# Zelana-Labs/zelana

Measured on AMD Instinct MI355X. Metric: BN254 G1 MSM Mpoint-scalar/s + L2 proofs/sec at 1/2/4/8 MI355X, higher is better.
Workload: dtype u32

## Files before the change

### zelana_amd/csrc/dev_io.h

```cpp
#pragma once
#include <hip/hip_runtime.h>

#include "ff.h"

namespace zk {

__device__ __forceinline__ Fe ld_fe(const uint32_t* p) {
  uint4 a = reinterpret_cast<const uint4*>(p)[0];
  uint4 b = reinterpret_cast<const uint4*>(p)[1];
  uint32_t w[8] = {a.x, a.y, a.z, a.w, b.x, b.y, b.z, b.w};
  return unpack(w);
}
__device__ __forceinline__ void st_fe(uint32_t* p, const Fe& f) {
  uint32_t w[8];
  pack(w, f);
  reinterpret_cast<uint4*>(p)[0] = make_uint4(w[0], w[1], w[2], w[3]);
  reinterpret_cast<uint4*>(p)[1] = make_uint4(w[4], w[5], w[6], w[7]);
}
__device__ __forceinline__ Fe ldc_fe(const uint32_t* c) {
  uint32_t w[8];
#pragma unroll
  for (int i = 0; i < 8; i++) w[i] = c[i];
  return unpack(w);
}

}
```

### zelana_amd/csrc/ec.h

```cpp
#pragma once
#include "ff.h"

#if defined(__HIPCC__) || defined(__HIP__)
#define ZK_HD_NOINLINE __host__ __device__ __noinline__
#else
#define ZK_HD_NOINLINE inline
#endif

namespace zk {


template <class F>
struct Aff {
  typename F::T x, y;
};
template <class F>
struct Xyzz {
  typename F::T x, y, zz, zzz;
};

template <class F>
ZK_HD Xyzz<F> xyzz_inf() {
  Xyzz<F> r;
  r.x = F::zero();
// ... 190 lines not shown
  r.zzz = f2_mul_n(p.zzz, ppp);
  return r;
}

template <class P = FqP>
ZK_HD Xyzz<FqOps> xyzz_add_g1(const Xyzz<FqOps>& p, const Xyzz<FqOps>& q) {
  if (xyzz_is_inf(p)) return q;
  if (xyzz_is_inf(q)) return p;
  Fe u1 = mul<P>(p.x, q.zz);
  Fe u2 = mul<P>(q.x, p.zz);
  Fe s1 = mul<P>(p.y, q.zzz);
  Fe s2 = mul<P>(q.y, p.zzz);
  Fe pp_ = subk<P, 2>(u2, u1);
  Fe ny1 = subk<P, 2>(fe_zero(), s1);
  Fe rr = add_lazy(s2, ny1);
  Fe pp = sqr<P>(pp_);
  if (is_zero<P>(pp)) {
    Fe rn = reduce8<P>(subk<P, 2>(s2, s1));
    if (is_zero<P>(rn)) return xyzz_dbl(p);
    return xyzz_inf<FqOps>();
  }
  Fe ppp = mul<P>(pp_, pp);
  Fe qq = mul<P>(u1, pp);
  Fe t = add_lazy(add_lazy(ppp, qq), qq);
  Xyzz<FqOps> r;
  Fe x = subk<P, 6>(sqr<P>(rr), t);
  Fe qx = subk<P, 8>(qq, x);
  r.y = mul2<P>(rr, qx, ny1, ppp);
  r.x = reduce8<P>(x);
  r.zz = mul<P>(mul<P>(p.zz, q.zz), pp);
  r.zzz = mul<P>(mul<P>(p.zzz, q.zzz), ppp);
  return r;
}
ZK_HD Xyzz<Fq2Ops> xyzz_add_g2(const Xyzz<Fq2Ops>& p, const Xyzz<Fq2Ops>& q) {
  if (xyzz_is_inf(p)) return q;
  if (xyzz_is_inf(q)) return p;
  Fe2 u1 = f2_mul_n(p.x, q.zz), u2 = f2_mul_n(q.x, p.zz);
  Fe2 s1 = f2_mul_n(p.y, q.zzz), s2 = f2_mul_n(q.y, p.zzz);
  Fe2 pp_ = {subk<FqPn, 2>(u2.c0, u1.c0), subk<FqPn, 2>(u2.c1, u1.c1)};
  Fe2 rr = {subk<FqPn, 2>(s2.c0, s1.c0), subk<FqPn, 2>(s2.c1, s1.c1)};
  Fe2 pp = f2_sqr_n(pp_);
  if (f2_is_zero(pp)) {
    if (is_zero<FqPn>(reduce8<FqPn>(rr.c0)) && is_zero<FqPn>(reduce8<FqPn>(rr.c1))) return xyzz_dbl(p);
    return xyzz_inf<Fq2Ops>();
  }
  Fe2 r2 = f2_sqr_n(rr);
  Fe2 ppp = f2_mul_n(pp_, pp), qq = f2_mul_n(u1, pp);
  Xyzz<Fq2Ops> r;
  r.x.c0 = reduce8<FqPn>(subk<FqPn, 6>(r2.c0, add_lazy(add_lazy(ppp.c0, qq.c0), qq.c0)));
  r.x.c1 = reduce8<FqPn>(subk<FqPn, 6>(r2.c1, add_lazy(add_lazy(ppp.c1, qq.c1), qq.c1)));
  Fe2 qx = {subk<FqPn, 2>(qq.c0, r.x.c0), subk<FqPn, 2>(qq.c1, r.x.c1)};
  Fe ny0 = subk<FqPn, 2>(fe_zero(), s1.c0), ny1 = subk<FqPn, 2>(fe_zero(), s1.c1);
  Fe nqx1 = subk<FqPn, 4>(fe_zero(), qx.c1), nppp1 = subk<FqPn, 2>(fe_zero(), ppp.c1);
  r.y.c0 = mul4<FqPn>(rr.c0, qx.c0, rr.c1, nqx1, ny0, ppp.c0, ny1, nppp1);
  r.y.c1 = mul4<FqPn>(rr.c0, qx.c1, rr.c1, qx.c0, ny0, ppp.c1, ny1, ppp.c0);
  r.zz = f2_mul_n(f2_mul_n(p.zz, q.zz), pp);
  r.zzz = f2_mul_n(f2_mul_n(p.zzz, q.zzz), ppp);
  return r;
}

ZK_HD Fe fq_cneg(const Fe& y, bool neg_) {
  Fe n = subk<FqP, 2>(fe_zero(), y);
  Fe r;
#pragma unroll
  for (int i = 0; i < NL; i++) r.v[i] = neg_ ? n.v[i] : y.v[i];
  return r;
// ... 38 lines not shown
```

### zelana_amd/csrc/groth16.hip

```cpp
#include <string.h>

#include <algorithm>
#include <unordered_map>
#include <vector>

#include "dev_io.h"
#include "ec.h"
#include "fq_sqrt.h"
#include "r1cs_row.h"
#include "zkmi_internal.h"

struct zkmi_pk {
  zkmi_ctx* ctx;
  uint64_t n = 0, num_instance = 0, num_witness = 0;
  uint32_t log_n = 0;
  uint64_t alpha_g1[8], beta_g1[8], delta_g1[8];
  uint64_t beta_g2[16], gamma_g2[16], delta_g2[16];
  std::vector<uint64_t> gamma_abc;
  uint64_t a0[8], b1_0[8], b2_0[16];
  zkmi_bases *a_query = nullptr, *b_g1_query = nullptr, *b_g2_query = nullptr, *h_query_rev = nullptr,
             *l_query = nullptr;
  zkmi_bases *b_g1_c = nullptr, *b_g2_c = nullptr;
  uint32_t* d_bidx = nullptr;
  size_t nb_c = 0;
// ... 123 lines not shown
  Aff<Fq2Ops> P = {x, y};
  Xyzz<Fq2Ops> acc = xyzz_inf<Fq2Ops>();
  for (int bit = 253; bit >= 0; bit--) {
    acc = xyzz_dbl(acc);
    if ((FR_MOD64_G[bit >> 6] >> (bit & 63)) & 1) acc = xyzz_madd(acc, P);
  }
  if (!xyzz_is_inf(acc)) {
    atomicOr(bad, 2u);
    return;
  }
  st_fe(o, canon_q(x.c0));
  st_fe(o + 8, canon_q(x.c1));
  st_fe(o + 16, canon_q(y.c0));
  st_fe(o + 24, canon_q(y.c1));
}

__global__ void __launch_bounds__(256) k_permute_rev(const uint32_t* __restrict__ in, uint32_t logn, size_t cnt,
                                                     uint32_t* __restrict__ out) {
  size_t p = blockIdx.x * (size_t)blockDim.x + threadIdx.x;
  if (p >= cnt) return;
  size_t src = logn ? (__brev((uint32_t)p) >> (32 - logn)) : 0;
  for (int k = 0; k < 16; k++) out[p * 16 + k] = in[src * 16 + k];
}

__global__ void __launch_bounds__(256) k_to_mont_fr(const uint32_t* __restrict__ z, size_t n, uint32_t* __restrict__ zm,
                                                    size_t zstr = 0) {
  size_t i = blockIdx.x * (size_t)blockDim.x + threadIdx.x;
  if (i >= n) return;
  z += (size_t)blockIdx.y * zstr;
  zm += (size_t)blockIdx.y * n * 8;
  st_fe(zm + i * 8, to_mont<FrP>(ld_fe(z + i * 8)));
}
constexpr uint32_t MATVEC_SHORT = 8;
__device__ __forceinline__ Fe fe_shfl_xor(const Fe& a, int m) {
  Fe r;
#pragma unroll
  for (int i = 0; i < NL; i++) r.v[i] = (uint32_t)__shfl_xor((int)a.v[i], m, 64);
  return r;
}
__device__ __forceinline__ Fe fr_sum_reduce(Fe a) {
#pragma unroll
  for (int i = 0; i < NL - 1; i++) {
    a.v[i + 1] += a.v[i] >> 29;
    a.v[i] &= LMASK;
  }
  return reduce_q32<FrP>(a);
}
template <bool DICT>
__device__ __forceinline__ Fe mv_term(uint64_t k, const uint64_t* __restrict__ col, const uint32_t* __restrict__ val,
                                      const uint2* __restrict__ cv, const uint32_t* __restrict__ coef,
                                      const uint32_t* __restrict__ zm, const uint32_t* __restrict__ zc) {
  if constexpr (DICT) {
    const uint2 e = cv[k];
    Fe t = ld_fe(zc + (size_t)e.x * 8);
    if (e.y) t = mul<FrP>(ld_fe(coef + (size_t)e.y * 8), t);
    return t;
  } else {
    return mul<FrP>(ld_fe(val + k * 8), ld_fe(zm + col[k] * 8));
  }
}
template <bool DICT, class RP>
__global__ void __launch_bounds__(256) k_matvec(const RP* __restrict__ rowptr, const uint64_t* __restrict__ col,
                                                const uint32_t* __restrict__ val, const uint2* __restrict__ cv,
                                                const uint32_t* __restrict__ coef, const uint32_t* __restrict__ zm,
                                                const uint32_t* __restrict__ zc, size_t m, size_t l, size_t n,
                                                int is_a, const uint32_t* __restrict__ lrow, uint32_t nlong, int g,
                                                uint32_t nsb, uint32_t* __restrict__ out, size_t zstr,
                                                size_t zmstr) {
  zc += (size_t)blockIdx.y * zstr;
  if (!DICT) zm += (size_t)blockIdx.y * zmstr;
  out += (size_t)blockIdx.y * n * 8;
  if (blockIdx.x < nsb) {
// ... 1720 lines not shown
```

### zelana_amd/csrc/msm.hip

```cpp
#include <stdarg.h>
#include <stdlib.h>
#include <stdio.h>
#include <string.h>

#include <algorithm>
#include <string>
#include <type_traits>
#include <utility>
#include <vector>
#include <chrono>

#include "dev_io.h"
#include "ec.h"
#include "zkmi_internal.h"

namespace zk {

#define ZK_TAIL_WAVE() __builtin_amdgcn_s_setprio(3)

struct G1T {
  using F = FqOps;
  using P = FqP;
  static constexpr int CW = 8;
  static constexpr int PW = 16;
// ... 28 lines not shown

template <class G>
__device__ __forceinline__ Aff<typename G::F> ld_aff(const uint32_t* bases, uint32_t idx) {
  const uint32_t* p = bases + (size_t)idx * G::PW;
  Aff<typename G::F> a;
  a.x = Io<typename G::F>::ld(p);
  a.y = Io<typename G::F>::ld(p + G::CW);
  return a;
}
template <class G>
__device__ __forceinline__ Xyzz<typename G::F> ld_xyzz(const uint32_t* p) {
  using F = typename G::F;
  Xyzz<F> r;
  r.x = Io<F>::ld(p);
  r.y = Io<F>::ld(p + G::CW);
  r.zz = Io<F>::ld(p + 2 * G::CW);
  r.zzz = Io<F>::ld(p + 3 * G::CW);
  return r;
}
template <class G>
__device__ __forceinline__ void st_xyzz(uint32_t* p, const Xyzz<typename G::F>& v) {
  using F = typename G::F;
  Io<F>::st(p, v.x);
  Io<F>::st(p + G::CW, v.y);
  Io<F>::st(p + 2 * G::CW, v.zz);
  Io<F>::st(p + 3 * G::CW, v.zzz);
}


template <class G>
__device__ __forceinline__ Xyzz<typename G::F> br_add(const Xyzz<typename G::F>& p, const Xyzz<typename G::F>& q) {
  if constexpr (G::CW == 8) return xyzz_add_g1<typename G::P>(p, q);
  else return xyzz_add_g2(p, q);
}

__host__ __device__ constexpr int msm_windows(int c) { return (254 + c - 1) / c + ((254 % c) == 0 ? 1 : 0); }

template <int C, bool BAL>
struct WinLayout {
  static constexpr int W = msm_windows(C);
  static constexpr int A = BAL ? (254 - W * (C - 1) > 0 ? 254 - W * (C - 1) : 0) : W;
  static_assert(A >= 0 && A <= W && (!BAL || A < W), "balanced layout");
  static constexpr int width(int w) { return w < A ? C : C - 1; }
  static constexpr int offset(int w) { return w <= A ? w * C : A * C + (w - A) * (C - 1); }
};

template <int C, bool BAL = false>
__device__ __forceinline__ void scalar_digits(const uint32_t* __restrict__ scalars, size_t i, int32_t* d) {
  uint4 a = reinterpret_cast<const uint4*>(scalars)[2 * i];
  uint4 b = reinterpret_cast<const uint4*>(scalars)[2 * i + 1];
  uint32_t s[9] = {a.x, a.y, a.z, a.w, b.x, b.y, b.z, b.w & 0x3FFFFFFFu, 0};
  using L = WinLayout<C, BAL>;
  constexpr int W = L::W;
  uint32_t carry = 0;
#pragma unroll
  for (int w = 0; w < W; w++) {
      const int bit = L::offset(w), wi = bit >> 5, sh = bit & 31, wd = L::width(w);
    const uint32_t half = 1u << (wd - 1);
    uint64_t v64 = (((uint64_t)s[wi + 1 < 9 ? wi + 1 : 8]) << 32) | s[wi < 9 ? wi : 8];
    uint32_t v = (uint32_t)(v64 >> sh) & ((1u << wd) - 1);
    v += carry;
    if (w < W - 1 && v > half) {
      d[w] = (int32_t)v - (int32_t)(1u << wd);
      carry = 1;
    } else {
      d[w] = (int32_t)v;
// ... 1157 lines not shown
                   uint32_t tskip, uint32_t* __restrict__ buckets, uint32_t* __restrict__ xpts) {
  acc_items_body<G2T>(items, nover, nmain, sval, bases, tn, tskip, buckets, xpts);
}

__global__ void __launch_bounds__(256) k_items_place(const uint4* __restrict__ stage, uint32_t NLO, uint32_t cap,
                                                     const uint32_t* __restrict__ ghist, uint32_t* __restrict__ gcur,
                                                     uint4* __restrict__ items, uint32_t nmain) {
  ZK_TAIL_WAVE();
  __shared__ uint32_t lh[ITEM_CAP_MAX + 1], lstart[ITEM_CAP_MAX + 1], base[ITEM_CAP_MAX + 1], tmp[4];
  const uint32_t h = blockIdx.x;
  const uint4* st = stage + (size_t)h * NLO;
  for (uint32_t c = threadIdx.x; c <= cap; c += 256) lh[c] = 0;
  __syncthreads();
  for (uint32_t x = threadIdx.x; x < NLO; x += 256) {
    const uint4 it = st[x];
    atomicAdd(&lh[min(it.y - it.x, cap)], 1u);
  }
  __syncthreads();
  block_prefix<256>(cap + 1, [&](uint32_t k) { return lh[cap - k]; }, lstart, tmp);
  block_prefix<256>(cap + 1, [&](uint32_t k) { return ghist[cap - k]; }, base, tmp);
  for (uint32_t k = threadIdx.x; k <= cap; k += 256) {
    const uint32_t c = cap - k;
    if (lh[c]) base[k] += atomicAdd(&gcur[c], lh[c]);
  }
  __syncthreads();
  for (uint32_t x = threadIdx.x; x < NLO; x += 256) {
    const uint4 it = st[x];
    const uint32_t k = cap - min(it.y - it.x, cap);
    const uint32_t dst = base[k] + (x - lstart[k]);
    if (dst < nmain) items[dst] = it;
  }
}

template <class G, bool CHUNKED = false>
__global__ void __launch_bounds__(256) k_split_combine(const uint4* __restrict__ split,
                                                       const uint32_t* __restrict__ nsplit,
                                                       const uint32_t* __restrict__ xpts,
                                                       uint32_t* __restrict__ buckets) {
  ZK_TAIL_WAVE();
  using F = typename G::F;
  constexpr int XW = 4 * G::CW;
  constexpr uint32_t BIG = 256;
  __shared__ Xyzz<F> sh[4][32];
  __shared__ uint4 spl[4];
  const uint32_t ns = *nsplit;
  const uint32_t wave = threadIdx.x >> 6, lane = threadIdx.x & 63;
  for (uint32_t base = blockIdx.x * 4; base < ns; base += gridDim.x * 4) {
    if (lane == 0) spl[wave] = base + wave < ns ? split[base + wave] : make_uint4(0, 0, 0, 0);
    __syncthreads();
    uint32_t mxs = 0;
    for (int w = 0; w < 4; w++) mxs = max(mxs, spl[w].z <= BIG ? spl[w].z : 0u);
    const uint32_t nload0 = (mxs + 63) / 64;
    uint32_t lev0 = 0;
    while ((1u << lev0) < min(mxs, 64u)) lev0++;
    const uint4 mine = spl[wave];
    const bool small = mine.z <= BIG;
    Xyzz<F> v = xyzz_inf<F>();
    int ph = 0;
    uint32_t st0 = 0;
    uint32_t nload = nload0, lev = lev0, cross = 0, stride = 64;
    uint4 cur = mine;
    bool mine_in = small;
    for (uint32_t step = 0;; step++) {
      uint32_t k = step - st0;
      if (k >= nload + lev + cross) {
        if (ph == 0) {
          if (small && mine.z && lane == 0) st_xyzz<G>(buckets + (size_t)mine.x * XW, v);
        } else if (threadIdx.x == 0) {
          st_xyzz<G>(buckets + (size_t)cur.x * XW, v);
        }
        v = xyzz_inf<F>();
        int w = ph;
        while (w < 4 && spl[w].z <= BIG) w++;
        if (w >= 4) break;
        ph = w + 1;
        cur = spl[w];
        mine_in = true;
        st0 = step;
        k = 0;
// ... 151 lines not shown
    if (!first_open) {
      ykey[2 * t + 1] = first_key;
      yvalid[2 * t + 1] = 0;
    }
    if (!last_open || (first_key == last_key && first_open)) {
      ykey[2 * t + 2] = last_key;
      yvalid[2 * t + 2] = 0;
    }
    if (t == 0) {
      ykey[0] = first_key;
      yvalid[0] = 0;
    }
  }
  if (!head) return;
  const bool left_open = r == 0 && first_open;
  const bool right_open = key == last_key && last_open;
  if (left_open || right_open) {
    const uint32_t slot = left_open ? 2 * t + 1 : 2 * t + 2;
    ykey[slot] = key;
    yvalid[slot] = has;
    if (has) {
      st_xyzz<G>(ypts + (size_t)slot * XW, v);
      atomicOr(any_open, 1u);
    }
  } else if (has) {
    st_xyzz<G>(buckets + (size_t)key * XW, v);
  }
}


__device__ __forceinline__ uint32_t insert_bit(uint32_t t, int bit) {
  return (((t >> bit) << (bit + 1)) | (1u << bit) | (t & ((1u << bit) - 1)));
}
#define ZK_BR_WPE 4
#ifndef ZK_BR_MINW
#define ZK_BR_MINW 1
#endif

template <class G, bool BITS>
__global__ void __launch_bounds__(256) __attribute__((amdgpu_waves_per_eu(ZK_BR_MINW, ZK_BR_WPE))) k_msm_br(const uint32_t* __restrict__ src0, const uint32_t* __restrict__ src1,
                                                const uint32_t* __restrict__ bstart, int lb, int hb, int W, int sr,
                                                int sc, int sb, int segt, uint32_t* __restrict__ out0,
                                                uint32_t* __restrict__ out1) {
  ZK_TAIL_WAVE();
  using F = typename G::F;
  constexpr int XW = 4 * G::CW;
  __shared__ Xyzz<F> sh[4][32];
  const int bb = lb + hb;
  const uint32_t wave = threadIdx.x >> 6, lane = threadIdx.x & 63;
  const uint32_t job = blockIdx.x * 4 + wave;
  const uint32_t nrow = ((uint32_t)W << hb) * sr, ncol = ((uint32_t)W << lb) * sc;
  const uint32_t njobs = BITS ? (uint32_t)W * (bb + 1) * sb : nrow + ncol;
  const bool live = job < njobs;
  const uint32_t* src = src0;
  uint32_t cnt = 0, stride = 1, bucket0 = 0, t0 = 0;
  int bit = -1, seg = 1;
  uint32_t* dst = nullptr;
  bool canon = false;
  if (live) {
    if (!BITS) {
      if (job < nrow) {
        uint32_t rh = job / sr, g = job % sr, w = rh >> hb, h = rh & ((1u << hb) - 1);
        cnt = (1u << lb) / sr;
        bucket0 = (w << bb) + (h << lb) + g * cnt;
        stride = 1;
        dst = out0 + (size_t)job * XW;
      } else {
        uint32_t jj = job - nrow, cl = jj / sc, g = jj % sc, w = cl >> lb, l = cl & ((1u << lb) - 1);
        cnt = (1u << hb) / sc;
        bucket0 = (w << bb) + ((g * cnt) << lb) + l;
        stride = 1u << lb;
        dst = out1 + (size_t)jj * XW;
      }
      src = src0 + (size_t)bucket0 * XW;
    } else {
      const uint32_t wj = job / sb;
      t0 = (job % sb) * (uint32_t)segt;
      uint32_t w = wj / (bb + 1), j = wj % (bb + 1);
      if ((int)j < lb) {
        src = src1 + (((size_t)w << lb) * sc) * XW;
        cnt = (1u << (lb - 1)) * sc;
        bit = (int)j;
        seg = sc;
      } else if ((int)j < bb) {
        src = src0 + (((size_t)w << hb) * sr) * XW;
        cnt = (1u << (hb - 1)) * sr;
        bit = (int)j - lb;
        seg = sr;
      } else {
        src = src0 + (((size_t)w << hb) * sr) * XW;
        cnt = (1u << hb) * sr;
        seg = sr;
      }
      dst = out0 + (size_t)job * XW;
      canon = true;
    }
  }
  const uint32_t nload = BITS ? (uint32_t)segt / 64 : 256 / 64;
  const uint32_t tend = BITS ? min(cnt, t0 + (uint32_t)segt) : cnt;
  Xyzz<F> v = xyzz_inf<F>();
  for (uint32_t step = 0; step < nload + 6; step++) {
    Xyzz<F> q;
    bool act = false;
    if (step < nload) {
      uint32_t t = t0 + lane + 64u * step;
      if (live && t < tend) {
        uint32_t e = BITS ? (bit < 0 ? t : insert_bit(t / seg, bit) * seg + t % seg) : t * stride;
        bool nonempty = BITS ? true : bstart[bucket0 + e + 1] > bstart[bucket0 + e];
        if (nonempty) {
          q = ld_xyzz<G>(src + (size_t)e * XW);
          act = true;
        }
      }
    } else {
      uint32_t sz = 32u >> (step - nload);
      if (lane >= sz && lane < 2 * sz) sh[wave][lane - sz] = v;
      __syncthreads();
      if (lane < sz) {
        q = sh[wave][lane];
        act = !xyzz_is_inf(q);
      }
    }
    if (act) v = xyzz_is_inf(v) ? q : br_add<G>(v, q);
    if (step >= nload) __syncthreads();
  }
  if (live && lane == 0) {
    if (canon) {
      v.x = Io<F>::canon(v.x);
      v.y = Io<F>::canon(v.y);
      v.zz = Io<F>::canon(v.zz);
      v.zzz = Io<F>::canon(v.zzz);
    }
    st_xyzz<G>(dst, v);
  }
}

template <class G>
__global__ void __launch_bounds__(256) __attribute__((amdgpu_waves_per_eu(ZK_BR_MINW, ZK_BR_WPE))) k_msm_br_strip(const uint32_t* __restrict__ buckets,
                                                      const uint32_t* __restrict__ bstart, int lb, int hb, int W,
                                                      int sr, int sc, int mc, uint32_t* __restrict__ outC,
                                                      uint32_t* __restrict__ outD) {
  ZK_TAIL_WAVE();
  using F = typename G::F;
  constexpr int XW = 4 * G::CW;
  __shared__ Xyzz<F> sh[4][32];
  const int bb = lb + hb;
  const uint32_t wave = threadIdx.x >> 6, lane = threadIdx.x & 63;
  const uint32_t job = blockIdx.x * 4 + wave;
  const uint32_t nrow = ((uint32_t)W << hb) * sr, ncol = ((uint32_t)W << lb) * sc;
  const uint32_t cpw = 64u / (uint32_t)mc;
  const bool row_wave = job < nrow;
  const uint32_t m = row_wave ? 64u : (uint32_t)mc;
  const uint32_t sub = lane & (m - 1), lslot = (lane / m) * (m / 2);
  bool live = false;
  uint32_t len = 0, stride = 1, bucket0 = 0;
  uint32_t* dst = nullptr;
  if (row_wave) {
    const uint32_t rh = job / sr, g = job % sr, w = rh >> hb, h = rh & ((1u << hb) - 1);
    live = true;
    len = (1u << lb) / sr;
    bucket0 = (w << bb) + (h << lb) + g * len;
    stride = 1;
    dst = outC + (size_t)job * XW;
  } else {
    const uint32_t jj = (job - nrow) * cpw + lane / m;
    if (jj < ncol) {
      const uint32_t cl = jj / sc, g = jj % sc, w = cl >> lb, l = cl & ((1u << lb) - 1);
      live = true;
      len = (1u << hb) / sc;
      bucket0 = (w << bb) + ((g * len) << lb) + l;
      stride = 1u << lb;
      dst = outD + (size_t)jj * XW;
    }
  }
  const uint32_t L = (len + m - 1) / m;
  const uint32_t Lr = (((1u << lb) / sr) + 63) >> 6, Lc = (((1u << hb) / sc) + mc - 1) / mc;
  const uint32_t Lmax = Lr > Lc ? Lr : Lc;
  Xyzz<F> v = xyzz_inf<F>();
  for (uint32_t step = 0; step < Lmax + 6; step++) {
    Xyzz<F> q;
    bool act = false;
    if (step < Lmax) {
      const uint32_t t = sub * L + step;
      if (live && step < L && t < len) {
        const uint32_t b = bucket0 + t * stride;
        if (bstart[b + 1] > bstart[b]) {
          q = ld_xyzz<G>(buckets + (size_t)b * XW);
          act = true;
        }
      }
    } else {
      const uint32_t sz = 32u >> (step - Lmax);
      if (sz < m && sub >= sz && sub < 2 * sz) sh[wave][lslot + sub - sz] = v;
      __syncthreads();
      if (sz < m && sub < sz) {
        q = sh[wave][lslot + sub];
        act = !xyzz_is_inf(q);
      }
    }
    if (act) v = xyzz_is_inf(v) ? q : br_add<G>(v, q);
    if (step >= Lmax) __syncthreads();
  }
  if (live && sub == 0) st_xyzz<G>(dst, v);
}


__constant__ uint32_t G2B_C0[8] = {0x24a138e5u, 0x3267e6dcu, 0x59dbefa3u, 0xb5b4c5e5u,
                                   0x1be06ac3u, 0x81be1899u, 0xceb8aaaeu, 0x2b149d40u};
__constant__ uint32_t G2B_C1[8] = {0x85c315d2u, 0xe4a2bd06u, 0xe52d1852u, 0xa74fa084u,
                                   0xeed8fdf4u, 0xcd2cafadu, 0x3af0fed4u, 0x009713b0u};

template <class G>
__global__ void __launch_bounds__(256) k_bases_convert(const uint32_t* __restrict__ in, size_t n,
                                                       uint32_t* __restrict__ out, uint32_t* __restrict__ bad) {
  using F = typename G::F;
  size_t i = blockIdx.x * (size_t)blockDim.x + threadIdx.x;
  if (i >= n) return;
  const uint32_t* p = in + i * G::PW;
  uint32_t o = 0;
  for (int k = 0; k < G::PW; k++) o |= p[k];
  uint32_t* q = out + i * G::PW;
  if (o == 0) {
    for (int k = 0; k < G::PW; k++) q[k] = 0;
    q[G::PW - 1] = 0x80000000u;
    return;
  }
  if constexpr (G::CW == 8) {
    Fe x = to_mont<FqP>(ld_fe(p)), y = to_mont<FqP>(ld_fe(p + 8));
    Fe b = to_mont<FqP>(Fe{{3, 0, 0, 0, 0, 0, 0, 0, 0}});
    Fe lhs = sqr<FqP>(y), rhs = add<FqP>(mul<FqP>(sqr<FqP>(x), x), b);
    if (!eq<FqP>(lhs, rhs)) atomicOr(bad, 1u);
    st_fe(q, reduce<FqP>(x));
    st_fe(q + 8, reduce<FqP>(y));
  } else {
// ... 782 lines not shown
  auto scan = [&](uint32_t* a, size_t len, uint32_t* total) {
    uint32_t nb = (uint32_t)((len + 1023) / 1024);
    k_scan_blocks<<<nb, 256, 0, st>>>(a, (uint32_t)len, a, bsums);
    k_scan_top<<<1, 1024, 0, st>>>(bsums, nb, total);
    k_scan_add<<<(unsigned)((len + 255) / 256), 256, 0, st>>>(a, (uint32_t)len, bsums, nullptr);
  };
  const uint32_t ne = (uint32_t)P.ne;
  k_rs_p1_count<<<nc1, RS_THREADS, NH * 4, st>>>(digits, Mmax, ne, P.B, NH, lob, C1, nc1, cnt1);
  scan(cnt1, len1, &tot[0]);
  k_rs_p1_scatter<4096><<<nc1, RS_THREADS, rs_scatter_lds(NH, 4096), st>>>(digits, Mmax, ne, P.B, NH, lob, C1, nc1,
                                                                           cnt1, okey, oval);
  k_rs_tiles<<<1, 1024, 0, st>>>(cnt1, nc1, NH, &tot[0], C2, binstart, tstart);
  const uint32_t g2 = ((T2max + 7) / 8) * 8;
  k_rs_p2_count<<<g2, RS_THREADS, (1u << lob) * 4, st>>>(okey, binstart, tstart, NH, lob, C2, T2max, cnt2);
  scan(cnt2, len2, &tot[1]);
  k_rs_bstart<<<(P.K + 256) / 256, 256, 0, st>>>(cnt2, binstart, tstart, NH, lob, P.K, bstart);
  const uint32_t NLO = 1u << lob;
#define ZK_P2(ST, T) \
  k_rs_p2_scatter<ST, T><<<g2, T, rs_scatter_lds(NLO, ST, T), st>>>(okey, oval, binstart, tstart, NH, lob, C2, T2max, cnt2, sval)
  if (rs_scatter_lds(NLO, 8192, 1024) <= 160 * 1024) ZK_P2(8192, 1024);
  else ZK_P2(4096, 1024);
#undef ZK_P2
  ZK_HIP(hipGetLastError());
  *out_sval = sval;
  *out_bstart = bstart;
  return 0;
}

struct BrGeom {
  int mode;
  int sr, sc, sb, segt;
  int mc = 64;
};
static BrGeom br_geom(const MsmPlan& P, bool g2, bool pipelined) {
#ifndef ZK_BR_FOLD_G1
#define ZK_BR_FOLD_G1 8
#endif
  const int fold = g2 || pipelined ? 16 : ZK_BR_FOLD_G1;
  BrGeom g;
  g.mode = P.hb >= 9 ? 1 : 0;
  g.segt = 256;
  const int segb = g.mode == 1 ? 64 * fold : 256;
  g.sr = (1 << P.lb) > segb ? (1 << P.lb) / segb : 1;
  g.sc = (1 << P.hb) > segb ? (1 << P.hb) / segb : 1;
  const int lenc = (1 << P.hb) / g.sc;
  g.mc = 64;
  while (g.mc > 1 && lenc / g.mc < fold) g.mc >>= 1;
  const uint32_t maxterms = std::max((1u << P.hb) * g.sr, (1u << (P.lb - 1)) * g.sc);
  g.sb = (int)((maxterms + g.segt - 1) / g.segt);
  return g;
}

constexpr size_t SHARD_PAYLOAD_WORDS = 36864;
static uint32_t shard_sig0(int g2, int c, int bb, bool wmode = false) {
  return 0x5A000000u | ((uint32_t)wmode << 17) | ((uint32_t)g2 << 16) | ((uint32_t)c << 8) | (uint32_t)bb;
}
__global__ void k_put_words(uint32_t* __restrict__ dst, uint32_t w0, uint32_t w1, uint32_t w2, uint32_t w3) {
  if (threadIdx.x < 4) dst[threadIdx.x] = threadIdx.x == 0 ? w0 : threadIdx.x == 1 ? w1 : threadIdx.x == 2 ? w2 : w3;
}

static int msm_queue_handover(zkmi_ctx* ctx, MsmLane* lane, hipStream_t st, zkmi_msm_job* job, uint32_t* d_buf,
                              size_t words) {
  ZK_HIP(hipEventCreateWithFlags(&job->done, hipEventDisableTiming));
  if (!job->comm) {
    job->host_words = words;
    ZK_TRY(ctx_pinned_get(ctx, words * 4, (void**)&job->host));
    job->st = st;
    ZK_HIP(hipMemcpyAsync(job->host, d_buf + SHARD_STATUS_WORDS, words * 4, hipMemcpyDeviceToHost, st));
    ZK_HIP(hipEventRecord(job->done, st));
    job->done_rec = true;
    return 0;
  }
  const int nr = job->comm->nranks;
  const bool empty = words == 0;
  k_put_words<<<1, 64, 0, st>>>(d_buf, 0u, shard_sig0(job->g2, empty ? 0 : job->c, empty ? 0 : job->bb, job->wmode),
                                empty ? 0u : (uint32_t)job->sb,
                                empty ? 0u : (uint32_t)job->W | ((uint32_t)job->w0 << 16));
  ZK_HIP(hipGetLastError());
  const size_t width = empty || job->wmode ? SHARD_PAYLOAD_WORDS : SHARD_STATUS_WORDS + words;
  if (job->comm->kind == ZKMI_COMM_RCCL) {
    uint32_t* gathered;
    ZK_TRY(lane->ws.get("msm_gathered", (size_t)nr * SHARD_PAYLOAD_WORDS * 4, (void**)&gathered));
// ... 98 lines not shown
                                                                                                  xpts, buckets);
      ZK_HIP(hipGetLastError());
    } else {
    if (K <= CUTSUM_COOP_K)
      k_msm_cutsum_coop<GS><<<(unsigned)(((size_t)K * 16 + 255) / 256), 256, 0, st>>>(bstart, K, L, buckets, xvalid,
                                                                                   xpts, &flags[0]);
    else
      k_msm_cutsum<G><<<(K + 255) / 256, 256, 0, st>>>(bstart, K, L, buckets, xvalid, xpts, &flags[0]);
    uint32_t cur_len = (uint32_t)xl;
    for (int level = 1; cur_len > 1; level++) {
      if (level >= 63) {
        set_error("msm: segmented reduction schedule too deep");
        return ZKMI_EINVAL;
      }
      const bool coop = level > 1 && K <= CUTSUM_COOP_K;
      uint32_t Ll = level == 1 ? 2 : 16;
      uint32_t nc = (cur_len + Ll - 1) / Ll;
      if (coop)
        k_msm_accN_coop<GS><<<(unsigned)(((size_t)nc * 16 + 255) / 256), 256, 0, st>>>(
            xkey, xvalid, xpts, cur_len, nc, buckets, ykey, yvalid, ypts, &flags[level - 1], &flags[level]);
      else
        k_msm_accN<G><<<(nc + 255) / 256, 256, 0, st>>>(xkey, xvalid, xpts, cur_len, Ll, nc, buckets, ykey, yvalid,
                                                        ypts, &flags[level - 1], &flags[level]);
      std::swap(xkey, ykey);
      std::swap(xvalid, yvalid);
      std::swap(xpts, ypts);
      cur_len = nc == 1 ? 1 : 2 * nc + 1;
    }
    ZK_HIP(hipGetLastError());
    }
  }
  hipStream_t brs = st;
  uint32_t *Cb, *Db, *sums;
  const BrGeom bg = br_geom(P, G::CW != 8, ctx->msm_lanes > 1 && !job->comm);
  const int sr = bg.sr, sc = bg.sc, sb = bg.sb;
  ZK_TRY(ws.get("msm_C", (size_t)W * (1u << hb) * sr * XW * 4, (void**)&Cb));
  ZK_TRY(ws.get("msm_D", (size_t)W * (1u << lb) * sc * XW * 4, (void**)&Db));
  const size_t sum_words = (size_t)W * (bb + 1) * sb * XW;
  ZK_TRY(ws.get("msm_sums", std::max(sum_words + SHARD_STATUS_WORDS, job->comm ? SHARD_PAYLOAD_WORDS : 0) * 4,
                (void**)&sums));
  if (!(debug_skip() & 4)) {
    ScopedKernelTimer tm(ctx, "msm_bucket_reduce", brs);
    uint32_t jobs2 = (uint32_t)W * (bb + 1) * sb;
    if (bg.mode == 1) {
      const uint32_t nrow = (uint32_t)W * ((1u << hb) * sr), ncol = (uint32_t)W * ((1u << lb) * sc);
      const uint32_t cpw = 64u / (uint32_t)bg.mc;
      const uint32_t jobs1 = nrow + (ncol + cpw - 1) / cpw;
      k_msm_br_strip<GB><<<(jobs1 + 3) / 4, 256, 0, brs>>>(buckets, bstart, lb, hb, W, sr, sc, bg.mc, Cb, Db);
    } else {
      uint32_t jobs1 = (uint32_t)W * (((1u << hb) * sr) + ((1u << lb) * sc));
      auto br1 = K <= CUTSUM_COOP_K ? k_msm_br<GS, false> : k_msm_br<G, false>;
      br1<<<(jobs1 + 3) / 4, 256, 0, brs>>>(buckets, nullptr, bstart, lb, hb, W, sr, sc, sb, 256, Cb, Db);
    }
    auto br2 = K <= CUTSUM_COOP_K ? k_msm_br<GS, true> : k_msm_br<GB, true>;
    br2<<<(jobs2 + 3) / 4, 256, 0, brs>>>(Cb, Db, nullptr, lb, hb, W, sr, sc, sb, bg.segt,
                                          sums + SHARD_STATUS_WORDS, nullptr);
    ZK_HIP(hipGetLastError());
  }
  job->sb = sb;
  return msm_queue_handover(ctx, lane, brs, job, sums, sum_words);
}

static int msm_acc_any(zkmi_ctx* ctx, MsmLane* lane, const MsmPlan& P, const zkmi_bases* tb, size_t offset, size_t n,
                       const uint32_t* sval, const uint32_t* bstart, zkmi_msm_job* job) {
  if (ctx->acc_gate && tb == ctx->acc_gate_set) ZK_HIP(hipStreamWaitEvent(lane->st, ctx->acc_gate, 0));
  return tb->g2 ? msm_acc_phase<G2T>(ctx, lane, P, tb, offset, n, sval, bstart, job)
                : msm_acc_phase<G1T>(ctx, lane, P, tb, offset, n, sval, bstart, job);
// ... 416 lines not shown
```

Measured before the change: 948.3.

## Split G1 point additions across lane pairs in bucket-reduce tree reductions

Adds a cooperative XYZZ G1 addition in which two lanes each compute half of the field multiplications and swap intermediates through cross-lane shuffles. This replaces the shared-memory halving tree in the split-combine and bucket-reduce kernels, so both lanes of a pair do useful work and the per-level barriers go away. It also adds an optional 128-term segment size for bit-pattern reductions when the extra host-side adds stay small. The cost is many shuffles per addition and more code paths that must handle the infinity and doubling cases correctly.

```diff
diff --git a/zelana_amd/csrc/dev_io.h b/zelana_amd/csrc/dev_io.h
--- a/zelana_amd/csrc/dev_io.h
+++ b/zelana_amd/csrc/dev_io.h
@@ -17,6 +17,12 @@
   reinterpret_cast<uint4*>(p)[0] = make_uint4(w[0], w[1], w[2], w[3]);
   reinterpret_cast<uint4*>(p)[1] = make_uint4(w[4], w[5], w[6], w[7]);
 }
+__device__ __forceinline__ Fe fe_shfl_xor(const Fe& a, int m) {
+  Fe r;
+#pragma unroll
+  for (int i = 0; i < NL; i++) r.v[i] = (uint32_t)__shfl_xor((int)a.v[i], m, 64);
+  return r;
+}
 __device__ __forceinline__ Fe ldc_fe(const uint32_t* c) {
   uint32_t w[8];
 #pragma unroll
diff --git a/zelana_amd/csrc/ec.h b/zelana_amd/csrc/ec.h
--- a/zelana_amd/csrc/ec.h
+++ b/zelana_amd/csrc/ec.h
@@ -246,6 +246,62 @@
   r.zzz = mul<P>(mul<P>(p.zzz, q.zzz), ppp);
   return r;
 }
+#ifndef ZK_BOUND
+#define ZK_BOUND(a, k) ((void)0)
+#endif
+ZK_HD Fe fe_sel(bool c, const Fe& a, const Fe& b) {
+  Fe r;
+#pragma unroll
+  for (int i = 0; i < NL; i++) r.v[i] = c ? a.v[i] : b.v[i];
+  return r;
+}
+template <class P = FqP, class X>
+ZK_HD Xyzz<FqOps> xyzz_add_g1_pair(const Xyzz<FqOps>& my, bool role1, bool live, X&& xchg) {
+  ZK_BOUND(my.x, 2);
+  ZK_BOUND(my.y, 2);
+  ZK_BOUND(my.zz, 2);
+  ZK_BOUND(my.zzz, 2);
+  const Fe ozz = xchg(my.zz), ozzz = xchg(my.zzz);
+  if (live && (fe_is_zero_raw(my.zz) || fe_is_zero_raw(ozz))) {
+    const Fe ox = xchg(my.x), oy = xchg(my.y);
+    if (fe_is_zero_raw(my.zz)) return Xyzz<FqOps>{ox, oy, ozz, ozzz};
+    return my;
+  }
+  const Fe u = mul<P>(my.x, ozz);
+  const Fe s = mul<P>(my.y, ozzz);
+  const Fe z12 = mul<P>(fe_sel(role1, my.zzz, my.zz), fe_sel(role1, ozzz, ozz));
+  const Fe ou = xchg(u), os = xchg(s);
+  const Fe u1 = fe_sel(role1, ou, u), s1 = fe_sel(role1, os, s);
+  const Fe pp_ = subk<P, 2>(fe_sel(role1, u, ou), u1);
+  const Fe rr = subk<P, 2>(fe_sel(role1, s, os), s1);
+  ZK_BOUND(pp_, 4);
+  ZK_BOUND(rr, 4);
+  const Fe sq = sqr<P>(fe_sel(role1, rr, pp_));
+  const Fe pp = fe_sel(role1, xchg(sq), sq);
+  ZK_BOUND(pp, 2);
+  if (live && is_zero<P>(pp)) {
+    const Fe oz = xchg(z12);
+    if (is_zero<P>(reduce8<P>(rr))) return xyzz_dbl(Xyzz<FqOps>{u1, s1, fe_sel(role1, oz, z12), fe_sel(role1, z12, oz)});
+    return xyzz_inf<FqOps>();
+  }
+  const Fe m5 = mul<P>(fe_sel(role1, u1, pp_), pp);
+  const Fe ppp = fe_sel(role1, xchg(m5), m5);
+  ZK_BOUND(ppp, 2);
+  const Fe m6 = mul<P>(z12, fe_sel(role1, ppp, pp));
+  const Fe t = add_lazy(add_lazy(ppp, m5), m5);
+  const Fe x = subk<P, 6>(sq, t);
+  const Fe qx = subk<P, 8>(m5, x);
+  ZK_BOUND(x, 8);
+  ZK_BOUND(qx, 10);
+  const Fe m7 = mul<P>(fe_sel(role1, rr, s1), fe_sel(role1, qx, ppp));
+  const Fe ox = xchg(x), o7 = xchg(m7), o6 = xchg(m6);
+  Xyzz<FqOps> r;
+  r.x = reduce8<P>(ox);
+  r.y = sub<P>(o7, m7);
+  r.zz = m6;
+  r.zzz = o6;
+  return r;
+}
 ZK_HD Xyzz<Fq2Ops> xyzz_add_g2(const Xyzz<Fq2Ops>& p, const Xyzz<Fq2Ops>& q) {
   if (xyzz_is_inf(p)) return q;
   if (xyzz_is_inf(q)) return p;
diff --git a/zelana_amd/csrc/groth16.hip b/zelana_amd/csrc/groth16.hip
--- a/zelana_amd/csrc/groth16.hip
+++ b/zelana_amd/csrc/groth16.hip
@@ -179,12 +179,6 @@
   st_fe(zm + i * 8, to_mont<FrP>(ld_fe(z + i * 8)));
 }
 constexpr uint32_t MATVEC_SHORT = 8;
-__device__ __forceinline__ Fe fe_shfl_xor(const Fe& a, int m) {
-  Fe r;
-#pragma unroll
-  for (int i = 0; i < NL; i++) r.v[i] = (uint32_t)__shfl_xor((int)a.v[i], m, 64);
-  return r;
-}
 __device__ __forceinline__ Fe fr_sum_reduce(Fe a) {
 #pragma unroll
   for (int i = 0; i < NL - 1; i++) {
diff --git a/zelana_amd/csrc/msm.hip b/zelana_amd/csrc/msm.hip
--- a/zelana_amd/csrc/msm.hip
+++ b/zelana_amd/csrc/msm.hip
@@ -84,6 +84,15 @@
 __device__ __forceinline__ Xyzz<typename G::F> br_add(const Xyzz<typename G::F>& p, const Xyzz<typename G::F>& q) {
   if constexpr (G::CW == 8) return xyzz_add_g1<typename G::P>(p, q);
   else return xyzz_add_g2(p, q);
+}
+
+template <class G>
+__device__ __forceinline__ void br_pair_level(Xyzz<FqOps>& v, uint32_t sub, uint32_t sz) {
+  const bool in = sub < 2 * sz, role1 = (sub & sz) != 0;
+  const int fin = !xyzz_is_inf(v);
+  const bool ofin = __shfl_xor(fin, (int)sz, 64) != 0;
+  if (!__any(in && !role1 && ofin)) return;
+  v = xyzz_add_g1_pair<typename G::P>(v, role1, in, [sz](const Fe& a) { return fe_shfl_xor(a, (int)sz); });
 }
 
 __host__ __device__ constexpr int msm_windows(int c) { return (254 + c - 1) / c + ((254 % c) == 0 ? 1 : 0); }
@@ -1307,19 +1316,71 @@
   }
 }
 
+template <class G, bool CHUNKED>
+__device__ __forceinline__ void split_combine_pairs(const uint4* __restrict__ split, const uint32_t* __restrict__ nsplit,
+    const uint32_t* __restrict__ xpts, uint32_t* __restrict__ buckets) {
+  ZK_TAIL_WAVE();
+  using F = typename G::F;
+  constexpr int XW = 4 * G::CW;
+  constexpr uint32_t BIG = 256;
+  __shared__ uint4 spl[4];
+  const uint32_t ns = *nsplit;
+  const uint32_t wave = threadIdx.x >> 6, lane = threadIdx.x & 63;
+  __shared__ Xyzz<F> xw[3];
+  for (uint32_t base = blockIdx.x * 4; base < ns; base += gridDim.x * 4) {
+    if (lane == 0) spl[wave] = base + wave < ns ? split[base + wave] : make_uint4(0, 0, 0, 0);
+    __syncthreads();
+    for (int ph = 0; ph <= 4; ph++) {
+      const bool big = ph > 0;
+      const uint4 cur = spl[big ? ph - 1 : wave];
+      if (big ? cur.z <= BIG : (cur.z > BIG || cur.z == 0)) continue;
+      const uint32_t idx = big ? threadIdx.x : lane, stride = big ? 256u : 64u;
+      Xyzz<F> v = xyzz_inf<F>();
+#pragma unroll 1
+      for (uint32_t k = 0; k * stride < cur.z; k++) {
+        const uint32_t pc = idx + stride * k;
+        if (pc < cur.z) {
+          const uint32_t slot = CHUNKED ? (pc == 0 ? 2 * cur.y + 2 : 2 * (cur.y + pc) + 1) : cur.y + pc;
+          const Xyzz<F> q = ld_xyzz<G>(xpts + (size_t)slot * XW);
+          if (!xyzz_is_inf(q)) v = xyzz_is_inf(v) ? q : br_add<G>(v, q);
+        }
+      }
+      uint32_t nlev = 0;
+      while ((1u << nlev) < min(cur.z, 64u)) nlev++;
+#pragma unroll 1
+      for (uint32_t lvl = 0; lvl < nlev + (big ? 2u : 0u); lvl++) {
+        if (lvl == nlev) {
+          if (wave > 0 && lane == 0) xw[wave - 1] = v;
+          __syncthreads();
+          if (wave == 0 && lane >= 1 && lane < 4) v = xw[lane - 1];
+        }
+        const uint32_t sz = lvl < nlev ? (1u << (nlev - 1)) >> lvl : 2u >> (lvl - nlev);
+        if (lvl < nlev || wave == 0) br_pair_level<G>(v, lane, sz);
+      }
+      if (big) __syncthreads();
+      if (lane == 0 && (!big || wave == 0)) st_xyzz<G>(buckets + (size_t)cur.x * XW, v);
+    }
+    __syncthreads();
+  }
+}
+
 template <class G, bool CHUNKED = false>
 __global__ void __launch_bounds__(256) k_split_combine(const uint4* __restrict__ split,
                                                        const uint32_t* __restrict__ nsplit,
                                                        const uint32_t* __restrict__ xpts,
                                                        uint32_t* __restrict__ buckets) {
+  if constexpr (G::CW == 8) {
+    split_combine_pairs<G, CHUNKED>(split, nsplit, xpts, buckets);
+    return;
+  }
   ZK_TAIL_WAVE();
   using F = typename G::F;
   constexpr int XW = 4 * G::CW;
   constexpr uint32_t BIG = 256;
-  __shared__ Xyzz<F> sh[4][32];
   __shared__ uint4 spl[4];
   const uint32_t ns = *nsplit;
   const uint32_t wave = threadIdx.x >> 6, lane = threadIdx.x & 63;
+  __shared__ Xyzz<F> sh[4][32];
   for (uint32_t base = blockIdx.x * 4; base < ns; base += gridDim.x * 4) {
     if (lane == 0) spl[wave] = base + wave < ns ? split[base + wave] : make_uint4(0, 0, 0, 0);
     __syncthreads();
@@ -1537,6 +1598,7 @@
 __device__ __forceinline__ uint32_t insert_bit(uint32_t t, int bit) {
   return (((t >> bit) << (bit + 1)) | (1u << bit) | (t & ((1u << bit) - 1)));
 }
+constexpr int BR_PAIR_SEGT = 128;
 #define ZK_BR_WPE 4
 #ifndef ZK_BR_MINW
 #define ZK_BR_MINW 1
@@ -1550,7 +1612,6 @@
   ZK_TAIL_WAVE();
   using F = typename G::F;
   constexpr int XW = 4 * G::CW;
-  __shared__ Xyzz<F> sh[4][32];
   const int bb = lb + hb;
   const uint32_t wave = threadIdx.x >> 6, lane = threadIdx.x & 63;
   const uint32_t job = blockIdx.x * 4 + wave;
@@ -1604,30 +1665,59 @@
   const uint32_t nload = BITS ? (uint32_t)segt / 64 : 256 / 64;
   const uint32_t tend = BITS ? min(cnt, t0 + (uint32_t)segt) : cnt;
   Xyzz<F> v = xyzz_inf<F>();
-  for (uint32_t step = 0; step < nload + 6; step++) {
-    Xyzz<F> q;
-    bool act = false;
-    if (step < nload) {
-      uint32_t t = t0 + lane + 64u * step;
-      if (live && t < tend) {
-        uint32_t e = BITS ? (bit < 0 ? t : insert_bit(t / seg, bit) * seg + t % seg) : t * stride;
-        bool nonempty = BITS ? true : bstart[bucket0 + e + 1] > bstart[bucket0 + e];
-        if (nonempty) {
-          q = ld_xyzz<G>(src + (size_t)e * XW);
-          act = true;
+  constexpr bool PAIRS = G::CW == 8 && !(BITS && G::P::ASM);
+  if constexpr (PAIRS) {
+    auto term = [&](uint32_t t, Xyzz<F>& q) {
+      if (!(live && t < tend)) return false;
+      const uint32_t e = BITS ? (bit < 0 ? t : insert_bit(t / seg, bit) * seg + t % seg) : t * stride;
+      if (!BITS && !(bstart[bucket0 + e + 1] > bstart[bucket0 + e])) return false;
+      q = ld_xyzz<G>(src + (size_t)e * XW);
+      return true;
+    };
+    const bool pairf = BITS && segt == BR_PAIR_SEGT;
+    if (!pairf) {
+#pragma unroll 1
+      for (uint32_t step = 0; step < nload; step++) {
+        Xyzz<F> q;
+        if (term(t0 + lane + 64u * step, q)) v = xyzz_is_inf(v) ? q : br_add<G>(v, q);
+      }
+    }
+    const uint32_t n32 = pairf ? 3 : 1;
+#pragma unroll 1
+    for (uint32_t step = 0; step < n32 + 5; step++) {
+      if (pairf && step < n32 && (step == 0 || lane >= 32)) {
+        v = xyzz_inf<F>();
+        term(t0 + (step == 0 ? lane : (lane & 31) + 32 * (step + 1)), v);
+      }
+      br_pair_level<G>(v, lane, step < n32 ? 32u : 16u >> (step - n32));
+    }
+  } else {
+    __shared__ Xyzz<F> sh[4][32];
+    for (uint32_t step = 0; step < nload + 6; step++) {
+      Xyzz<F> q;
+      bool act = false;
+      if (step < nload) {
+        uint32_t t = t0 + lane + 64u * step;
+        if (live && t < tend) {
+          uint32_t e = BITS ? (bit < 0 ? t : insert_bit(t / seg, bit) * seg + t % seg) : t * stride;
+          bool nonempty = BITS ? true : bstart[bucket0 + e + 1] > bstart[bucket0 + e];
+          if (nonempty) {
+            q = ld_xyzz<G>(src + (size_t)e * XW);
+            act = true;
+          }
+        }
+      } else {
+        uint32_t sz = 32u >> (step - nload);
+        if (lane >= sz && lane < 2 * sz) sh[wave][lane - sz] = v;
+        __syncthreads();
+        if (lane < sz) {
+          q = sh[wave][lane];
+          act = !xyzz_is_inf(q);
         }
       }
-    } else {
-      uint32_t sz = 32u >> (step - nload);
-      if (lane >= sz && lane < 2 * sz) sh[wave][lane - sz] = v;
-      __syncthreads();
-      if (lane < sz) {
-        q = sh[wave][lane];
-        act = !xyzz_is_inf(q);
-      }
-    }
-    if (act) v = xyzz_is_inf(v) ? q : br_add<G>(v, q);
-    if (step >= nload) __syncthreads();
+      if (act) v = xyzz_is_inf(v) ? q : br_add<G>(v, q);
+      if (step >= nload) __syncthreads();
+    }
   }
   if (live && lane == 0) {
     if (canon) {
@@ -1648,7 +1738,6 @@
   ZK_TAIL_WAVE();
   using F = typename G::F;
   constexpr int XW = 4 * G::CW;
-  __shared__ Xyzz<F> sh[4][32];
   const int bb = lb + hb;
   const uint32_t wave = threadIdx.x >> 6, lane = threadIdx.x & 63;
   const uint32_t job = blockIdx.x * 4 + wave;
@@ -1680,31 +1769,49 @@
   }
   const uint32_t L = (len + m - 1) / m;
   const uint32_t Lr = (((1u << lb) / sr) + 63) >> 6, Lc = (((1u << hb) / sc) + mc - 1) / mc;
-  const uint32_t Lmax = Lr > Lc ? Lr : Lc;
   Xyzz<F> v = xyzz_inf<F>();
-  for (uint32_t step = 0; step < Lmax + 6; step++) {
-    Xyzz<F> q;
-    bool act = false;
-    if (step < Lmax) {
+  if constexpr (G::CW == 8) {
+    const uint32_t Lw = row_wave ? Lr : Lc;
+#pragma unroll 1
+    for (uint32_t step = 0; step < Lw; step++) {
       const uint32_t t = sub * L + step;
       if (live && step < L && t < len) {
         const uint32_t b = bucket0 + t * stride;
         if (bstart[b + 1] > bstart[b]) {
-          q = ld_xyzz<G>(buckets + (size_t)b * XW);
-          act = true;
+          const Xyzz<F> q = ld_xyzz<G>(buckets + (size_t)b * XW);
+          v = xyzz_is_inf(v) ? q : br_add<G>(v, q);
         }
       }
-    } else {
-      const uint32_t sz = 32u >> (step - Lmax);
-      if (sz < m && sub >= sz && sub < 2 * sz) sh[wave][lslot + sub - sz] = v;
-      __syncthreads();
-      if (sz < m && sub < sz) {
-        q = sh[wave][lslot + sub];
-        act = !xyzz_is_inf(q);
+    }
+#pragma unroll 1
+    for (uint32_t sz = m >> 1; sz; sz >>= 1) br_pair_level<G>(v, sub, sz);
+  } else {
+    __shared__ Xyzz<F> sh[4][32];
+    const uint32_t Lmax = Lr > Lc ? Lr : Lc;
+    for (uint32_t step = 0; step < Lmax + 6; step++) {
+      Xyzz<F> q;
+      bool act = false;
+      if (step < Lmax) {
+        const uint32_t t = sub * L + step;
+        if (live && step < L && t < len) {
+          const uint32_t b = bucket0 + t * stride;
+          if (bstart[b + 1] > bstart[b]) {
+            q = ld_xyzz<G>(buckets + (size_t)b * XW);
+            act = true;
+          }
+        }
+      } else {
+        const uint32_t sz = 32u >> (step - Lmax);
+        if (sz < m && sub >= sz && sub < 2 * sz) sh[wave][lslot + sub - sz] = v;
+        __syncthreads();
+        if (sz < m && sub < sz) {
+          q = sh[wave][lslot + sub];
+          act = !xyzz_is_inf(q);
+        }
       }
-    }
-    if (act) v = xyzz_is_inf(v) ? q : br_add<G>(v, q);
-    if (step >= Lmax) __syncthreads();
+      if (act) v = xyzz_is_inf(v) ? q : br_add<G>(v, q);
+      if (step >= Lmax) __syncthreads();
+    }
   }
   if (live && sub == 0) st_xyzz<G>(dst, v);
 }
@@ -2553,7 +2660,8 @@
   int sr, sc, sb, segt;
   int mc = 64;
 };
-static BrGeom br_geom(const MsmPlan& P, bool g2, bool pipelined) {
+constexpr uint32_t BR_PAIR_HOST_ADDS = 64;
+static BrGeom br_geom(const MsmPlan& P, bool g2, bool pipelined, bool pairbits = false) {
 #ifndef ZK_BR_FOLD_G1
 #define ZK_BR_FOLD_G1 8
 #endif
@@ -2569,6 +2677,13 @@
   while (g.mc > 1 && lenc / g.mc < fold) g.mc >>= 1;
   const uint32_t maxterms = std::max((1u << P.hb) * g.sr, (1u << (P.lb - 1)) * g.sc);
   g.sb = (int)((maxterms + g.segt - 1) / g.segt);
+  if (pairbits && !g2) {
+    const uint32_t sbp = (maxterms + BR_PAIR_SEGT - 1) / BR_PAIR_SEGT;
+    if ((uint32_t)P.W * (P.bb + 1) * (sbp - g.sb) <= BR_PAIR_HOST_ADDS) {
+      g.segt = BR_PAIR_SEGT;
+      g.sb = (int)sbp;
+    }
+  }
   return g;
 }
 
@@ -2733,7 +2848,10 @@
   }
   hipStream_t brs = st;
   uint32_t *Cb, *Db, *sums;
-  const BrGeom bg = br_geom(P, G::CW != 8, ctx->msm_lanes > 1 && !job->comm);
+#ifndef ZK_BR_PAIRBITS
+#define ZK_BR_PAIRBITS 1
+#endif
+  const BrGeom bg = br_geom(P, G::CW != 8, ctx->msm_lanes > 1 && !job->comm, ZK_BR_PAIRBITS && !job->comm && K <= CUTSUM_COOP_K);
   const int sr = bg.sr, sc = bg.sc, sb = bg.sb;
   ZK_TRY(ws.get("msm_C", (size_t)W * (1u << hb) * sr * XW * 4, (void**)&Cb));
   ZK_TRY(ws.get("msm_D", (size_t)W * (1u << lb) * sc * XW * 4, (void**)&Db));
```

Result: no change. 956.7 (median of 6 runs) (+0.9%).
